# JuliaParallel/DistributedArrays.jl

Hardware: NVIDIA H100
Metric: GB/s for map! and sum on Float32 DArray (higher is better)
Workload: dtype f32

## Files before the change

distributedarrays.jl_b200/_broadcast.py:

```python
from __future__ import annotations

import ctypes as C
import struct
from typing import Callable, List, Optional, Sequence, Tuple

import numpy as np

from builtins import any as builtins_any

from . import _lib
from ._darray import B200Array, DArray, dab_dtype, darray, makelocal
from .layout import shape_of
from .runtime import close_remote_reads, open_remote_reads, runtime

_RANK = {"bool": 0, "i32": 1, "i64": 2, "i128": 3, "f32": 4, "f64": 5}


class _TagTypes(dict):

    def __missing__(self, tag):
        raise _lib.UnsupportedError(_lib.ERR_UNSUPPORTED, f"values of type {tag} have no array element type on the GPU backend "
                                    "(Int128 is served as the value type of mapreduce(f, op, d) only)")


_NPT = _TagTypes({"bool": np.dtype(np.bool_), "i32": np.dtype(np.int32), "i64": np.dtype(np.int64), "f32": np.dtype(np.float32),
                  "f64": np.dtype(np.float64), "c64": np.dtype(np.complex64), "c128": np.dtype(np.complex128)})
_TAG = {v: k for k, v in _NPT.items()}
SLICE_TRACING = [0]
_CT = {"bool": "bool", "i32": "int", "i64": "long long", "i128": "i128", "f32": "float", "f64": "double", "c64": "jl_c64", "c128": "jl_c128"}
_COMP = {"c64": "f32", "c128": "f64"}
_CPLX_OF = {"f32": "c64", "f64": "c128"}


def is_ctag(t: str) -> bool:
    return t in _COMP

# ... 498 lines not shown
    for d in range(nd):
        o = int(out_shape[d])
        ext = [sh[d] for sh in shapes]
        for e, sh in zip(ext, arg_shapes):
            if e != o and e != 1:
                raise _lib.DimensionMismatch(_lib.ERR_DIM_MISMATCH, f"arrays could not be broadcast: {tuple(sh)} vs {tuple(out_shape)}")
        if o == 1:
            continue
        if groups:
            po, pext = groups[-1]
            if all((pe == po and e == o) or (pe == 1 and e == 1) for pe, e in zip(pext, ext)):
                groups[-1] = (po * o, [pe * e for pe, e in zip(pext, ext)])
                continue
        groups.append((o, ext))
    if not groups:
        groups = [(1, [1] * len(shapes))]
    return tuple(g[0] for g in groups), [tuple(g[1][k] for g in groups) for k in range(len(shapes))]


def _dense_strides(shape):
    s, out = 1, []
    for d in shape:
        out.append(s)
        s *= int(d)
    return out


class LocalArg:

    def __init__(self, arr: Optional[B200Array] = None, scalar=None, tag: str = "f64", temp: bool = False):
        self.arr, self.scalar, self.tag, self.temp = arr, scalar, tag, temp


def run_local(rt, expr: Expr, out: B200Array, largs: List[LocalArg]):
    n = out.size
    if n == 0:
        return
    out_tag = tag_of(out.dtype)
    full = [a for a in largs if a.arr is not None]
    same = all(a.arr.shape == out.shape or a.arr.size == n and _squeeze(a.arr.shape) == _squeeze(out.shape) for a in full)
    ctx = rt.ctx
    code = dab_dtype(out.dtype)
    rt.last_kernel = "fixed"
    cplx = uses_complex(expr) or builtins_any(is_ctag(a.tag) for a in largs)
    if same and not cplx and expr.jt == out_tag and out_tag != "bool":
        x0 = largs[0] if largs and largs[0].arr is not None and largs[0].tag == out_tag else None
        if x0 is not None and all(_only_arg0(expr)):
            ab = match_affine(expr)
            if ab is not None:
                a = np.asarray(ab[0], dtype=out.dtype)
                b = np.asarray(ab[1], dtype=out.dtype)
                _lib.call("dab_affine", ctx, code, C.c_void_p(out.ptr), C.c_void_p(x0.arr.ptr), C.c_void_p(a.ctypes.data),
                          C.c_void_p(b.ctypes.data), n)
                rt.last_kernel = "dab_affine"
                return
            if expr.op in _UN and _is_arg(expr.args[0], 0):
                _lib.call("dab_unary", ctx, code, _UN[expr.op], C.c_void_p(out.ptr), C.c_void_p(x0.arr.ptr), n)
                return
            if _is_arg(expr, 0):
                _lib.call("dab_unary", ctx, code, _lib.MAP_ID, C.c_void_p(out.ptr), C.c_void_p(x0.arr.ptr), n)
                return
        if expr.op in _BIN and len(expr.args) == 2 and not (expr.op == "div" and out_tag[0] != "f"):
            l, r = expr.args
            la = largs[l.val] if l.op == "arg" else None
            ra = largs[r.val] if r.op == "arg" else None

            def arr_ok(e, a):
                return e.op == "arg" and a is not None and a.arr is not None and a.tag == out_tag

            def sc_val(e, a):
                if e.op == "const" and e.jt == out_tag:
                    return e.val
                if e.op == "arg" and a is not None and a.arr is None and a.tag == out_tag:
                    return a.scalar
                return None

            if arr_ok(l, la) and arr_ok(r, ra):
                _lib.call("dab_binary", ctx, code, _BIN[expr.op], C.c_void_p(out.ptr), C.c_void_p(la.arr.ptr), C.c_void_p(ra.arr.ptr), n)
                return
            if arr_ok(l, la) and sc_val(r, ra) is not None:
                s = np.asarray(sc_val(r, ra), dtype=out.dtype)
                _lib.call("dab_binary_scalar", ctx, code, _BIN[expr.op], C.c_void_p(out.ptr), C.c_void_p(la.arr.ptr), C.c_void_p(s.ctypes.data), 0, n)
                return
            if arr_ok(r, ra) and sc_val(l, la) is not None:
                s = np.asarray(sc_val(l, la), dtype=out.dtype)
                _lib.call("dab_binary_scalar", ctx, code, _BIN[expr.op], C.c_void_p(out.ptr), C.c_void_p(ra.arr.ptr), C.c_void_p(s.ctypes.data), 1, n)
                return
    if expr.op == "const" and expr.jt == out_tag:
        v = np.asarray(expr.val, dtype=out.dtype)
        _lib.call("dab_fill", ctx, code, C.c_void_p(out.ptr), n, C.c_void_p(v.ctypes.data))
        return
    rt.last_kernel = "dab_broadcast_expr"
    if uses_tag(expr, "i128"):
        raise _lib.UnsupportedError(_lib.ERR_UNSUPPORTED, "Int128 values are served inside mapreduce(f, op, d) only, not in a broadcast")
    if expr.jt[0] == "f" and out_tag[0] not in "fc":
        raise _lib.UnsupportedError(_lib.ERR_UNSUPPORTED, f"broadcast of {expr.jt} values into a {out_tag} destination (InexactError semantics) is not served")
    if is_ctag(expr.jt) and not is_ctag(out_tag):
        raise _lib.UnsupportedError(_lib.ERR_UNSUPPORTED, f"broadcast of {expr.jt} values into a {out_tag} destination (InexactError semantics) is not served")
    expr, largs = split_c128_scalars(expr, largs)
    src = codegen(convert(expr, out_tag)).encode()
    oshape_nd, ashapes = tuple(out.shape), {k: tuple(a.arr.shape) for k, a in enumerate(largs) if a.arr is not None}
    if len(oshape_nd) > 4 or any(len(sh) > 4 for sh in ashapes.values()):
        keys = sorted(ashapes)
        oshape_nd, coll = collapse_dims(oshape_nd, [ashapes[k] for k in keys])
        ashapes = dict(zip(keys, coll))
    oshape = _pad4(oshape_nd)
    nargs = len(largs)
    if nargs > 8:
        raise _lib.UnsupportedError(_lib.ERR_UNSUPPORTED, "more than 8 broadcast arguments are not served")
    dts = (C.c_int32 * max(nargs, 1))()
    ptrs = (C.c_void_p * max(nargs, 1))()
    strides = (C.c_size_t * (4 * max(nargs, 1)))()
    scal = (C.c_uint64 * max(nargs, 1))()
    for k, a in enumerate(largs):
        dts[k] = dab_dtype(_NPT[a.tag])
        if a.arr is not None:
            ptrs[k] = a.arr.ptr
            ash = _pad4(ashapes[k])
            dense = _dense_strides(ash)
            for d in range(4):
                if ash[d] == oshape[d]:
                    strides[4 * k + d] = dense[d]
                elif ash[d] == 1:
                    strides[4 * k + d] = 0
                else:
                    raise _lib.DimensionMismatch(_lib.ERR_DIM_MISMATCH, f"arrays could not be broadcast: {a.arr.shape} vs {out.shape}")
        else:
            ptrs[k] = None
            scal[k] = struct.unpack("<Q", np.asarray(a.scalar, dtype=_NPT[a.tag]).tobytes().ljust(8, b"\0"))[0]
    _lib.call("dab_broadcast_expr", ctx, src, code, C.c_void_p(out.ptr), _lib.sz4(oshape), _lib.sz4(_dense_strides(oshape)), nargs, dts,
              ptrs, strides, scal)


def split_c128_scalars(expr: Expr, largs: List["LocalArg"]):
    ks = [k for k, a in enumerate(largs) if a.arr is None and a.tag == "c128"]
    if not ks:
        return expr, largs
    largs, sub = list(largs), {}
    for k in ks:
        z = complex(largs[k].scalar)
        largs[k] = LocalArg(None, z.real, "f64")
        largs.append(LocalArg(None, z.imag, "f64"))
        sub[k] = Expr("complex", (Expr("arg", (), "f64", k), Expr("arg", (), "f64", len(largs) - 1)), "c128")

    def rw(e: Expr) -> Expr:
        if e.op == "arg":
            return sub.get(e.val, e)
        return Expr(e.op, tuple(rw(a) for a in e.args), e.jt, e.val, e.weak) if e.args else e

    return rw(expr), largs


def _squeeze(shape):
    return tuple(s for s in shape if s != 1)


def _only_arg0(e: Expr):
    if e.op == "arg":
        yield e.val == 0
    elif e.op != "const":
        for a in e.args:
            yield from _only_arg0(a)


# ... 24 lines not shown

def _bcview(arg_dims: Sequence[int], I) -> Tuple:
    out = []
    for k, s in enumerate(arg_dims):
        if s == 1:
            out.append((1, 1))
        elif k < len(I):
            lo, hi = I[k]
            if not (1 <= lo and hi <= s):
                raise _lib.DimensionMismatch(_lib.ERR_DIM_MISMATCH, "broadcast view could not be constructed")
            out.append((lo, hi))
        else:
            out.append((1, s))
    return tuple(out)


def _localise(rt, a, I, pid) -> LocalArg:
    if isinstance(a, DArray):
        view = _bcview(a.dims, I)
        arr = makelocal(a, view, pid)
        return LocalArg(arr, None, tag_of(a.dtype), temp=arr is not a.chunks.get(pid))
    if isinstance(a, np.ndarray) and a.ndim > 0:
        view = _bcview(a.shape, I)
        sl = a[tuple(slice(lo - 1, hi) for lo, hi in view)]
        return LocalArg(B200Array.from_numpy(rt, sl), None, tag_of(a.dtype), temp=True)
    e = Expr.wrap(a.item() if isinstance(a, np.ndarray) else a)
    return LocalArg(None, e.val, e.jt)


def _remote_args(dest_layout, args) -> List[DArray]:
    return [a for a in args if isinstance(a, DArray) and not (a.layout.pids == dest_layout.pids and a.layout.indices == dest_layout.indices)]


def _broadcast_chunks(dest: DArray, expr: Expr, args) -> DArray:
    rt = dest.rt
    fenced = open_remote_reads(rt, _remote_args(dest.layout, args), "host")
    for pid, out in dest.chunks.items():
        I = dest.layout.localindices(pid)
        largs = [_localise(rt, a, I, pid) for a in args]
        run_local(rt, expr, out, largs)
        for la in largs:
            if la.temp and la.arr is not None:
                la.arr.free()
    close_remote_reads(rt, fenced, "host")
    return dest


def _materialise_views(args):
    from ._darray import SubDArray
    out, temps = [], []
    for a in args:
        if isinstance(a, SubDArray):
            a = a.to_darray()
            temps.append(a)
        out.append(a)
    return out, temps


def broadcast_into(dest: DArray, f: Callable, *args) -> DArray:
    args, _views = _materialise_views(args)
    try:
        return _broadcast_into(dest, f, *args)
    finally:
        for v in _views:
            v.close()


def _broadcast_into(dest: DArray, f: Callable, *args) -> DArray:
    shapes = [a.dims if isinstance(a, DArray) else (a.shape if isinstance(a, np.ndarray) else ()) for a in args]
    for shp in shapes:
        for k, s in enumerate(shp):
            want = dest.dims[k] if k < len(dest.dims) else 1
            if s != 1 and s != want:
                raise _lib.DimensionMismatch(_lib.ERR_DIM_MISMATCH, f"destination axes {dest.dims} are not compatible with source axes {tuple(shp)}")
    expr = trace(f, [_arg_tag(a) for a in args])
    return _broadcast_chunks(dest, expr, args)


def broadcast(f: Callable, *args, rt=None) -> DArray:
    args, _views = _materialise_views(args)
    try:
        return _broadcast(f, *args, rt=rt)
    finally:
        for v in _views:
            v.close()


def _broadcast(f: Callable, *args, rt=None) -> DArray:
    rt = rt or next((a.rt for a in args if isinstance(a, DArray)), None) or runtime()
    shapes = [a.dims if isinstance(a, DArray) else (a.shape if isinstance(a, np.ndarray) else ()) for a in args]
    dims = _bc_shape(shapes)
    expr = trace(f, [_arg_tag(a) for a in args])
    out_dt = _NPT[expr.jt]
    dest = darray(lambda I: B200Array.empty(rt, shape_of(I), out_dt), dims, dtype=out_dt, rt=rt)
    return _broadcast_chunks(dest, expr, args)


def copy(d: DArray) -> DArray:
    from ._darray import similar
    return _broadcast_into(similar(d), lambda x: x, d)


deepcopy = copy


def drandn(dims, procs=None, dist=None, dtype=np.float64, seed: int = 1234, rt=None) -> DArray:
    from ._darray import component_dtype, drand
    dt = np.dtype(dtype)
    if dt.kind == "c":
# ... 61 lines not shown
```

distributedarrays.jl_b200/_mapreduce.py:

```python
from __future__ import annotations

import builtins
import ctypes as C
import operator
from typing import Callable, Dict, Optional, Sequence, Tuple

import numpy as np

from . import _lib
from ._broadcast import Expr, broadcast, is_ctag, tag_of, trace, _NPT
from ._darray import B200Array, DArray, component_dtype, dab_dtype, is_complex, np_dtype
from .layout import Layout, collapse_for_region, ravel, shape_of, unravel
from .runtime import close_remote_reads, exchange_stacks, fence, grouped_exchange, open_remote_reads

_OPS = {"+": _lib.SUM, "add": _lib.SUM, "sum": _lib.SUM, "*": _lib.PROD, "mul": _lib.PROD, "prod": _lib.PROD, "max": _lib.MAX,
        "min": _lib.MIN}
_OPF = {operator.add: _lib.SUM, operator.mul: _lib.PROD, builtins.max: _lib.MAX, builtins.min: _lib.MIN, np.add: _lib.SUM,
        np.multiply: _lib.PROD, np.maximum: _lib.MAX, np.minimum: _lib.MIN}


def _op_code(op) -> int:
    if isinstance(op, str) and op in _OPS:
        return _OPS[op]
    if op in _OPF:
# ... 17 lines not shown
            code = {"abs": _lib.MAP_ABS, "abs2": _lib.MAP_ABS2, "neg": _lib.MAP_NEG, "isnan": _lib.MAP_ISNAN}.get(e.op)
            if code is not None:
                return code, None, e
        return None, None, e
    if e.jt == tag and len(e.args) == 1 and e.args[0].op == "arg":
        code = {"abs": _lib.MAP_ABS, "abs2": _lib.MAP_ABS2, "neg": _lib.MAP_NEG}.get(e.op)
        if code is not None:
            return code, None, e
    if e.op == "mul" and e.jt == tag and builtins.all(a.op == "arg" for a in e.args):
        return _lib.MAP_ABS2, None, e
    if e.op in _CMPMAP:
        l, r = e.args

        def unpromote(side, const):
            if side.op == "convert" and side.args[0].op == "arg" and side.args[0].jt == tag and const.op == "const":
                c = const.val
                if tag == "f32" and const.jt == "f64" and float(np.float32(c)) == c:
                    return side.args[0], Expr("const", (), tag, c)
                if tag in ("i32", "i64") and const.jt in ("i64",) and side.jt == "i64":
                    return side.args[0], Expr("const", (), tag, c) if -2**31 <= c < 2**31 or tag == "i64" else (side, const)
            return side, const

        l, r = unpromote(l, r)
        r, l = unpromote(r, l)
        if l.op == "arg" and r.op == "const" and l.jt == tag:
            return _CMPMAP[e.op], np.asarray(r.val, dtype=np.dtype(dtype)), e
        if r.op == "arg" and l.op == "const" and r.jt == tag:
            return _CMPMAP[_FLIP[e.op]], np.asarray(l.val, dtype=np.dtype(dtype)), e
    if e.op == "isnan" and e.args[0].op == "arg":
        return _lib.MAP_ISNAN, None, e
    return None, None, e


def _result_dtype(dtype, op: int, mapc: int) -> np.dtype:
    out = C.c_int32()
    _lib.check(_lib.lib().dab_reduce_result_dtype(dab_dtype(dtype), op, mapc, C.byref(out)))
    return np.dtype(np.int64) if out.value == _lib.I64 else np_dtype(out.value)




def _gather_slots(d: DArray, launch: Callable[[int, B200Array, int], None]) -> np.ndarray:
    rt = d.rt
    wpr = rt.workers_per_rank
    slots = B200Array.empty(rt, (16 * wpr,), np.uint8, temp=True)
    try:
        for pid, ch in d.chunks.items():
            launch(pid, ch, slots.ptr + 16 * ((pid - 1) % wpr))
        if rt.world > 1:
            allslots = B200Array.empty(rt, (16 * wpr * rt.world,), np.uint8, temp=True)
            _lib.call("dab_allgather", rt.ctx, C.c_void_p(slots.ptr), C.c_void_p(allslots.ptr), 16 * wpr)
            host = allslots.to_numpy()
            allslots.free()
        else:
            host = slots.to_numpy()
    finally:
        rt.sync()
        slots.free()
    return host.view(np.uint8)


def _fold(host: np.ndarray, pids: Sequence[int], rdt: np.dtype, op: int):
    vals = np.empty(len(pids), dtype=rdt)
    for i, pid in enumerate(pids):
        vals[i] = host[16 * (pid - 1):16 * (pid - 1) + rdt.itemsize].view(rdt)[0]
    out = np.zeros(1, dtype=rdt)
    rcode = _lib.I64 if rdt == np.dtype(np.int64) else dab_dtype(rdt)
    _lib.check(_lib.lib().dab_combine_ordered(rcode, op, C.c_void_p(vals.ctypes.data), len(pids), C.c_void_p(out.ctypes.data)))
    return out[0], vals

# ... 82 lines not shown
        _lib.call("dab_mapreduce_expr", rt.ctx, src, val_code, opc_k, ch.size, n, dts, ptrs, scal, C.c_void_p(slot_ptr))

    try:
        host = _gather_slots(d, launch)
    finally:
        for t in temps:
            t.free()
        close_remote_reads(rt, fenced, "host")
    if wide:
        vals = [_int128(host[16 * (pid - 1):16 * pid].tobytes()) for pid in d.layout.pids]
        res = fold128(vals, opc)
        return (res, vals) if return_partials else res
    res, vals = _fold(host, d.layout.pids, rdt, opc if opc != _lib.COUNT else _lib.SUM)
    return (res, vals) if return_partials else res


def _mapreduce_all(f, op, d: DArray, return_partials: bool = False, others: Sequence = ()):
    opc = op if isinstance(op, int) else _op_code(op)
    if others:
        expr = trace(f, [tag_of(d.dtype)] + [_arg_tag_of(a) for a in others])
        return _mapreduce_expr(expr, opc, d, others, return_partials)
    mapc, param, expr = classify_map(f, d.dtype)
    if is_complex(d.dtype) and mapc is not None and not _complex_served(opc, mapc):
        if mapc == _lib.MAP_ID and opc in (_lib.MAX, _lib.MIN):
            raise TypeError(f"MethodError: no method matching isless(::{d.dtype}, ::{d.dtype}) -- complex numbers are not ordered")
        mapc = None
        if expr is None:
            expr = trace(lambda z: z, [tag_of(d.dtype)])
    if mapc is None:
        return _mapreduce_expr(expr, opc, d, (), return_partials)
    _check_nonempty(d, opc)
    rt = d.rt
    pp = C.c_void_p(param.ctypes.data) if param is not None else None
    rdt = _result_dtype(d.dtype, opc, mapc)
    if rt.workers_per_rank == 1 and d.layout.pids == rt.workers() and not return_partials:
        ch = d.chunks[rt.myid()]
        out = np.zeros(2, dtype=np.uint64)
        _lib.call("dab_mapreduce_all", rt.ctx, dab_dtype(d.dtype), opc, mapc, pp, C.c_void_p(ch.ptr), ch.size, C.c_void_p(out.ctypes.data))
        return out.view(np.uint8)[:rdt.itemsize].view(rdt)[0]
    code = dab_dtype(d.dtype)
    host = _gather_slots(d, lambda pid, ch, slot: _lib.call("dab_reduce", rt.ctx, code, opc, mapc, pp, C.c_void_p(ch.ptr), ch.size, C.c_void_p(slot)))
    res, vals = _fold(host, d.layout.pids, rdt, opc)
    return (res, vals) if return_partials else res


def _complex_served(opc: int, mapc: int) -> bool:
    out = C.c_int32()
    return _lib.lib().dab_reduce_result_dtype(_lib.C64, opc, mapc, C.byref(out)) == _lib.OK


def _arg_tag_of(a) -> str:
    from ._broadcast import _arg_tag
    return _arg_tag(a)


def reduce(op, d: DArray, dims=None, init=None):
    return mapreduce(None, op, d, dims=dims, init=init)


def mapreduce(f: Optional[Callable], op, d: DArray, *ds, dims=None, init=None, _partials: bool = False):
    from ._darray import SubDArray
    if isinstance(d, Expr):
        from . import _slices
        if _slices.tracing():
            return _slices.reduce_of_slice(f, op, d, ds, dims, init)
    if isinstance(d, SubDArray):
        tmp = d.to_darray()
        try:
            return mapreduce(f, op, tmp, *ds, dims=dims, init=init, _partials=_partials)
        finally:
            if dims is None:
                tmp.close()
    if dims is None:
        if init is not None:
            raise _lib.UnsupportedError(_lib.ERR_UNSUPPORTED, "mapreduce(f, op, d; init) without dims falls back to scalar iteration in the reference; not served")
        return _mapreduce_all(f, op, d, _partials, ds)
    if ds:
        tmp = broadcast(f, d, *ds)
        try:
            return mapreducedim(None, op, tmp, dims, init)
        finally:
            tmp.close()
    return mapreducedim(f, op, d, dims, init)


def sum(d: DArray, f: Optional[Callable] = None, dims=None):
    return mapreduce(f, "+", d, dims=dims)


def prod(d: DArray, f: Optional[Callable] = None, dims=None):
    return mapreduce(f, "*", d, dims=dims)


def maximum(d: DArray, f: Optional[Callable] = None, dims=None):
    return mapreduce(f, "max", d, dims=dims)


def minimum(d: DArray, f: Optional[Callable] = None, dims=None):
    return mapreduce(f, "min", d, dims=dims)


def _pred_reduce(opc: int, d: DArray, f: Optional[Callable]):
    from ._darray import SubDArray
    if isinstance(d, SubDArray):
        tmp = d.to_darray()
        try:
            return _pred_reduce(opc, tmp, f)
        finally:
            tmp.close()
    if f is None:
        if d.dtype != np.dtype(np.bool_):
            raise TypeError("TypeError: non-boolean used in boolean context")
        return _mapreduce_all(None, opc, d)
    mapc, param, e = classify_map(f, d.dtype)
    if e is not None and e.jt != "bool":
        raise TypeError("TypeError: non-boolean used in boolean context")
    return _mapreduce_all(f, opc, d)


def _count_dims(d: DArray, f: Optional[Callable], dims) -> Tuple[DArray, int]:
    from ._broadcast import ifelse
    from ._darray import SubDArray
    if isinstance(d, SubDArray):
        tmp = d.to_darray()
        try:
            return _count_dims(tmp, f, dims)
        finally:
            tmp.close()
    if f is None and d.dtype != np.dtype(np.bool_):
        raise TypeError("TypeError: non-boolean used in boolean context")
    pred = (lambda x: x) if f is None else f
# ... 331 lines not shown
```

distributedarrays.jl_b200/csrc/dab_comm.cu:

```cuda
#include <dlfcn.h>
#include <nccl.h>

#include "dab_common.cuh"
#include "dab_scalar_ops.cuh"

namespace {

struct NcclApi {
    void* handle = nullptr;
    ncclResult_t (*GetUniqueId)(ncclUniqueId*) = nullptr;
    ncclResult_t (*CommInitRank)(ncclComm_t*, int, ncclUniqueId, int) = nullptr;
    ncclResult_t (*CommDestroy)(ncclComm_t) = nullptr;
    ncclResult_t (*AllGather)(const void*, void*, size_t, ncclDataType_t, ncclComm_t, cudaStream_t) = nullptr;
    ncclResult_t (*AllReduce)(const void*, void*, size_t, ncclDataType_t, ncclRedOp_t, ncclComm_t, cudaStream_t) = nullptr;
    ncclResult_t (*Send)(const void*, size_t, ncclDataType_t, int, ncclComm_t, cudaStream_t) = nullptr;
    ncclResult_t (*Recv)(void*, size_t, ncclDataType_t, int, ncclComm_t, cudaStream_t) = nullptr;
    ncclResult_t (*GroupStart)() = nullptr;
    ncclResult_t (*GroupEnd)() = nullptr;
    const char* (*GetErrorString)(ncclResult_t) = nullptr;
    const char* (*GetLastError)(ncclComm_t) = nullptr;
    bool ok = false;
    char why[256] = "";
};

NcclApi& nccl() {
    static NcclApi api;
    static bool tried = false;
    if (tried) return api;
    tried = true;
    const char* names[] = {"libnccl.so.2", "libnccl.so", nullptr};
    for (int i = 0; names[i] && !api.handle; ++i) api.handle = dlopen(names[i], RTLD_NOW | RTLD_GLOBAL);
    if (!api.handle) {
        snprintf(api.why, sizeof(api.why), "dlopen(libnccl.so.2) failed: %s", dlerror());
        return api;
// ... 149 lines not shown
        default: return dab_fail(ctx, DAB_ERR_ARG, "dab_allreduce: bad op %d", op);
    }
    DAB_NCCL(ctx, api.AllReduce(send_dev, recv_dev, count, dt, ro, (ncclComm_t)ctx->comm, ctx->stream));
    ctx->launches++;
    return DAB_OK;
}

int32_t dab_group_start(dab_ctx* ctx) {
    DAB_ENTER(ctx);
    NEED_COMM(ctx);
    DAB_NCCL(ctx, api.GroupStart());
    return DAB_OK;
}
int32_t dab_group_end(dab_ctx* ctx) {
    DAB_ENTER(ctx);
    NEED_COMM(ctx);
    DAB_NCCL(ctx, api.GroupEnd());
    ctx->launches++;
    return DAB_OK;
}
int32_t dab_send(dab_ctx* ctx, const void* send_dev, size_t nbytes, int32_t peer) {
    DAB_ENTER(ctx);
    NEED_COMM(ctx);
    DAB_NCCL(ctx, api.Send(send_dev, nbytes, ncclInt8, peer, (ncclComm_t)ctx->comm, ctx->stream));
    return DAB_OK;
}
int32_t dab_recv(dab_ctx* ctx, void* recv_dev, size_t nbytes, int32_t peer) {
    DAB_ENTER(ctx);
    NEED_COMM(ctx);
    DAB_NCCL(ctx, api.Recv(recv_dev, nbytes, ncclInt8, peer, (ncclComm_t)ctx->comm, ctx->stream));
    return DAB_OK;
}

int32_t dab_mapreduce_all(dab_ctx* ctx, int32_t dtype, int32_t op, int32_t map, const void* map_param, const void* x, size_t n,
                          void* out_host) {
    DAB_ENTER_NOFLUSH(ctx);
    int32_t rdt;
    if (!out_host || op == DAB_EXTREMA || dab_reduce_result_dtype(dtype, op, map, &rdt) != DAB_OK) {
        DAB_FLUSH(ctx);
        DAB_REQUIRE(ctx, out_host, DAB_ERR_ARG, "dab_mapreduce_all: null out");
        if (op == DAB_EXTREMA) return dab_fail(ctx, DAB_ERR_UNSUPPORTED, "dab_mapreduce_all: extrema combines through dab_reduce + dab_allgather");
        return dab_fail(ctx, DAB_ERR_ARG, "bad dtype/op");
    }
    const bool cplx = rdt == DAB_C64 || rdt == DAB_C128;
    if ((ctx->mbox_ranks > 1 || !ctx->comm || ctx->nranks == 1) && n > 0 && !cplx) {
        ctx->fuse_op = op;
        int32_t st = dab_reduce(ctx, dtype, op, map, map_param, x, n, ctx->result_slot);
        ctx->fuse_op = -1;
        if (st != DAB_OK) return st;
        DAB_CUDA(ctx, cudaStreamSynchronize(ctx->stream));
        const volatile unsigned long long* h = (const volatile unsigned long long*)ctx->host_slot;
        if (h[1] != 0) return dab_fail(ctx, DAB_ERR_NCCL, "fused combine timed out waiting for a peer's chunk result (did every rank call?)");
        unsigned long long bits = h[0];
        memset(out_host, 0, 8);
        memcpy(out_host, &bits, dab_dtype_size(rdt));
        return DAB_OK;
    }
    if (cplx && ctx->mbox_ranks > 1 && !ctx->comm) {
        DAB_FLUSH(ctx);
        return dab_fail(ctx, DAB_ERR_UNSUPPORTED, "dab_mapreduce_all: a complex result across %d ranks needs the NCCL communicator "
                        "(the mailbox combine carries 8-byte results)", ctx->mbox_ranks);
    }
    int32_t st = dab_reduce(ctx, dtype, op, map, map_param, x, n, ctx->result_slot);
    if (st != DAB_OK) return st;
    const int P = ctx->comm ? ctx->nranks : 1;
    const void* src = ctx->result_slot;
    if (P > 1) {
        NEED_COMM(ctx);
        DAB_NCCL(ctx, api.AllGather(ctx->result_slot, ctx->gather_slots, 16, ncclInt8, (ncclComm_t)ctx->comm, ctx->stream));
        ctx->launches++;
        src = ctx->gather_slots;
    }
    DAB_CUDA(ctx, cudaMemcpyAsync(ctx->host_slot, src, (size_t)P * 16, cudaMemcpyDeviceToHost, ctx->stream));
    DAB_CUDA(ctx, cudaStreamSynchronize(ctx->stream));
    unsigned char tmp[DAB_MAX_RANKS * 16];
    size_t es = dab_dtype_size(rdt);
    for (int i = 0; i < P; ++i) memcpy(tmp + (size_t)i * es, (const char*)ctx->host_slot + (size_t)i * 16, es);
    unsigned char res[16] = {0};
    st = dab_combine_ordered(rdt, op, tmp, (size_t)P, res);
    if (st != DAB_OK) return dab_fail(ctx, st, "%s", dab_last_error(nullptr));
    memset(out_host, 0, es > 8 ? es : 8);
    memcpy(out_host, res, es);
    return DAB_OK;
}
// ... 126 lines not shown
```

distributedarrays.jl_b200/csrc/dab_common.cuh:

```cuda
#pragma once
#include <cuda_runtime.h>

#include <cstdint>
#include <cstdio>
#include <cstring>

#include "../../include/dab200.h"

#define DAB_MAX_REDUCE_BLOCKS 262144
#define DAB_SLOT_BYTES 64
#define DAB_MAX_RANKS 64

struct dab_pending_affine {
    int active;
    int32_t dtype;
    void* y;
    const void* x;
    size_t n;
    unsigned char a[8], b[8];
};

struct dab_ctx {
    int device;
    int sm_count;
    cudaStream_t stream;
    void* block_partials;
    unsigned int* counter;
    void* result_slot;
    void* gather_slots;
    void* host_slot;
    void* dim_scratch;
    size_t dim_scratch_bytes;
    uint64_t launches;
    void* comm;
    int rank, nranks;
    void* mailbox;
    void** peer_mbox_dev;
    void* peer_mbox_host[DAB_MAX_RANKS];
    int mbox_ranks;
    unsigned long long mbox_seq;
    unsigned long long barrier_seq;
    int fuse_op;
    struct dab_alloc_cache* cache;
    void* sort_dev;
    size_t sort_dev_bytes;
    void* stage[2];
    cudaEvent_t stage_ev[2];
    void* sort_host;
    unsigned long long sort_epoch;
    long long opt_combine_timeout_ms;
    long long opt_gemm_kc;
    int opt_gemm_rawhi;
    int opt_gemm_simt;
    int opt_gemv_phase;
    int opt_gemv_t_cols;
    int opt_gemv_t_waves;
    int opt_ew_tma;
    dab_pending_affine pending;
    int defer_off;
    char err[512];
};

extern thread_local char dab_tls_err[512];

int32_t dab_fail(dab_ctx* ctx, int32_t status, const char* fmt, ...);
int32_t dab_fail_cuda(dab_ctx* ctx, cudaError_t e, const char* what, const char* file, int line);

#define DAB_CUDA(ctx, call)                                                             \
    do {                                                                                \
        cudaError_t e__ = (call);                                                       \
        if (e__ != cudaSuccess) return dab_fail_cuda((ctx), e__, #call, __FILE__, __LINE__); \
    } while (0)

#define DAB_REQUIRE(ctx, cond, status, ...)                          \
// ... 16 lines not shown
        if ((ctx) == nullptr) return dab_fail(nullptr, DAB_ERR_ARG, "null ctx"); \
        DAB_CUDA((ctx), cudaSetDevice((ctx)->device));                      \
        DAB_FLUSH(ctx);                                                     \
    } while (0)

#define DAB_ENTER_NOFLUSH(ctx)                                              \
    do {                                                                    \
        if ((ctx) == nullptr) return dab_fail(nullptr, DAB_ERR_ARG, "null ctx"); \
        DAB_CUDA((ctx), cudaSetDevice((ctx)->device));                      \
    } while (0)

#define DAB_LAUNCHED(ctx)                          \
    do {                                           \
        (ctx)->launches++;                         \
        DAB_CUDA((ctx), cudaGetLastError());       \
    } while (0)

static inline size_t dab_dtype_size(int32_t dt) {
    switch (dt) {
        case DAB_F32: return 4;
        case DAB_F64: return 8;
        case DAB_I32: return 4;
        case DAB_I64: return 8;
        case DAB_U8: return 1;
        case DAB_C64: return 8;
        case DAB_C128: return 16;
        default: return 0;
    }
}

#define DAB_MBOX_SLOT 32
#define DAB_MBOX_BARRIER_OFFSET (2 * DAB_MAX_RANKS * DAB_MBOX_SLOT)
#define DAB_MBOX_BYTES (DAB_MBOX_BARRIER_OFFSET + DAB_MAX_RANKS * 8)
struct FusedComm {
    void* const* peers;
    void* host_out;
    unsigned long long seq;
    unsigned long long timeout_ns;
    int rank, nranks, op;
};

__device__ __forceinline__ unsigned long long dab_globaltimer_ns() {
    unsigned long long t;
    asm volatile("mov.u64 %0, %globaltimer;" : "=l"(t));
    return t;
}
__device__ __forceinline__ int4 ld_stream(const int4* p) { return __ldcs(p); }
__device__ __forceinline__ void st_stream(int4* p, int4 v) { __stcs(p, v); }

template <typename T>
struct alignas(16) Pack {
    static constexpr int N = 16 / sizeof(T);
    T v[N];
};

template <typename T>
struct alignas(2 * sizeof(T)) Cplx {
    T re, im;
};

template <typename T>
__device__ __forceinline__ Pack<T> as_pack(int4 r) {
    Pack<T> p;
    memcpy(&p, &r, 16);
    return p;
}
template <typename T>
__device__ __forceinline__ int4 as_int4(const Pack<T>& p) {
    int4 r;
// ... 25 lines not shown
```

distributedarrays.jl_b200/csrc/dab_core.cu:

```cuda
#include <cstdarg>
#include <cstdlib>
#include <map>
#include <mutex>
#include <new>
#include <thread>
#include <unordered_map>

#include "dab_common.cuh"

thread_local char dab_tls_err[512] = "";

struct dab_alloc_cache {
    std::unordered_map<void*, size_t> live;
    std::multimap<size_t, void*> free_blocks;
    size_t cached_bytes = 0;
    static constexpr size_t kMaxBlock = 16ull << 30;
    static constexpr size_t kMaxCached = 32ull << 30;
};

int dab_resident_ctas(const void* kernel, int threads) {
    static std::mutex mu;
    static std::unordered_map<const void*, int> cache;
    std::lock_guard<std::mutex> lk(mu);
    auto it = cache.find(kernel);
// ... 75 lines not shown
    ctx->opt_gemv_t_waves = 4;
    ctx->opt_gemv_t_cols = 8;
    ctx->cache = new (std::nothrow) dab_alloc_cache();
#define INIT_CUDA(call)                                                     \
    do {                                                                    \
        cudaError_t e__ = (call);                                           \
        if (e__ != cudaSuccess) {                                           \
            int32_t st = dab_fail_cuda(nullptr, e__, #call, __FILE__, __LINE__); \
            delete ctx;                                                     \
            return st;                                                      \
        }                                                                   \
    } while (0)
    INIT_CUDA(cudaSetDevice(device));
    cudaDeviceProp prop;
    INIT_CUDA(cudaGetDeviceProperties(&prop, device));
    if (prop.major != 9 || prop.minor != 0) {
        delete ctx;
        return dab_fail(nullptr, DAB_ERR_UNSUPPORTED, "device %d is sm_%d%d; libdab200 is built for sm_90a only", device,
                        prop.major, prop.minor);
    }
    ctx->sm_count = prop.multiProcessorCount;
    INIT_CUDA(cudaStreamCreateWithFlags(&ctx->stream, cudaStreamNonBlocking));
    {
        cudaMemPool_t pool;
        INIT_CUDA(cudaDeviceGetDefaultMemPool(&pool, device));
        unsigned long long keep = ~0ull;
        INIT_CUDA(cudaMemPoolSetAttribute(pool, cudaMemPoolAttrReleaseThreshold, &keep));
    }
    INIT_CUDA(cudaMalloc(&ctx->block_partials, ((size_t)DAB_MAX_REDUCE_BLOCKS + DAB_MAX_REDUCE_BLOCKS / 256 + 16) * 16));
    INIT_CUDA(cudaMalloc((void**)&ctx->counter, (DAB_MAX_REDUCE_BLOCKS / 256 + 16) * 4));
    INIT_CUDA(cudaMemsetAsync(ctx->counter, 0, (DAB_MAX_REDUCE_BLOCKS / 256 + 16) * 4, ctx->stream));
    INIT_CUDA(cudaMalloc(&ctx->result_slot, DAB_SLOT_BYTES));
    INIT_CUDA(cudaMalloc(&ctx->gather_slots, (size_t)DAB_MAX_RANKS * 16));
    INIT_CUDA(cudaHostAlloc(&ctx->host_slot, (size_t)(DAB_MAX_RANKS + 2) * 16, cudaHostAllocDefault));
    INIT_CUDA(cudaStreamSynchronize(ctx->stream));
    memset(ctx->host_slot, 0, (size_t)(DAB_MAX_RANKS + 2) * 16);
#undef INIT_CUDA
    *out = ctx;
    return DAB_OK;
}

int32_t dab_comm_destroy(dab_ctx* ctx);
int32_t dab_mailbox_detach(dab_ctx* ctx);

int32_t dab_shutdown(dab_ctx* ctx) {
    if (!ctx) return DAB_OK;
    cudaSetDevice(ctx->device);
    const int32_t st = dab_flush_pending(ctx);
    cudaStreamSynchronize(ctx->stream);
    if (ctx->comm) dab_comm_destroy(ctx);
    cudaFree(ctx->block_partials);
    cudaFree(ctx->counter);
    cudaFree(ctx->result_slot);
    cudaFree(ctx->gather_slots);
    if (ctx->dim_scratch) cudaFree(ctx->dim_scratch);
    if (ctx->sort_dev) cudaFree(ctx->sort_dev);
    if (ctx->sort_host) cudaFreeHost(ctx->sort_host);
    for (int b = 0; b < 2; ++b)
        if (ctx->stage[b]) {
            cudaFreeHost(ctx->stage[b]);
            cudaEventDestroy(ctx->stage_ev[b]);
        }
    if (ctx->cache) {
        for (auto& kv : ctx->cache->free_blocks) cudaFree(kv.second);
        delete ctx->cache;
        ctx->cache = nullptr;
    }
    dab_mailbox_detach(ctx);
    cudaFreeHost(ctx->host_slot);
// ... 363 lines not shown
```

distributedarrays.jl_b200/csrc/dab_reduce.cu:

```cuda
#include <type_traits>

#include <cmath>

#include "dab_reduce_traits.cuh"

namespace {

constexpr int RD_UNROLL = 4;

struct NoStore {
    template <typename T>
    __device__ __forceinline__ void vec(Pack<T>&, size_t) const {}
    template <typename T>
    __device__ __forceinline__ T scalar(T v, size_t) const { return v; }
};
template <typename T>
struct AffineStore {
    AffineF<T> f;
    T* y;
    int4* yv;
    __device__ __forceinline__ void vec(Pack<T>& p, size_t i) const {
#pragma unroll
        for (int k = 0; k < Pack<T>::N; ++k) p.v[k] = f(p.v[k]);
        st_stream(yv + i, as_int4(p));
// ... 94 lines not shown
    v = block_reduce<R>(v, smem);
    if (threadIdx.x == 0) {
        counter[1 + g] = 0;
        gpartials[g] = v;
        __threadfence();
        unsigned int ticket = atomicAdd(counter, 1u);
        is_last = (ticket == ngroups - 1);
    }
    __syncthreads();
    if (!is_last) return;
    __threadfence();
    A fin = R::identity();
    for (unsigned int i = threadIdx.x; i < ngroups; i += RD_THREADS) fin = R::comb(fin, gpartials[i]);
    fin = block_reduce<R>(fin, smem);
    if (threadIdx.x == 0) {
        *counter = 0;
        if constexpr (std::is_arithmetic<A>::value) {
            Out res;
            if (finalize_mode == 1) res = (Out)(fin == (A)n_for_all);
            else if (finalize_mode == 2) res = (Out)(fin != (A)0);
            else res = (Out)fin;
            memcpy(out, &res, sizeof(Out));
            if (sizeof(Out) < 8) memset((char*)out + sizeof(Out), 0, 8 - sizeof(Out));
            A wide = fin;
            memcpy((char*)out + 8, &wide, sizeof(A));
            if (sizeof(A) < 8) memset((char*)out + 8 + sizeof(A), 0, 8 - sizeof(A));
            if (fc.host_out && fc.nranks <= 1) {
                unsigned long long bits = 0;
                memcpy(&bits, &res, sizeof(Out));
                volatile unsigned long long* h = reinterpret_cast<volatile unsigned long long*>(fc.host_out);
                h[0] = bits;
                h[1] = 0ull;
                __threadfence_system();
            }
        } else if constexpr (is_cplx<Out>::value) {
            using CT = decltype(Out::re);
            const Out res{(CT)fin.re, (CT)fin.im};
            memset(out, 0, 16);
            memcpy(out, &res, sizeof(Out));
        } else {
            memset(out, 0, 16);
            memcpy(out, &fin, sizeof(A));
        }
    }
    if constexpr (!std::is_arithmetic<Out>::value) return;
    else {
    if (fc.nranks <= 1) return;
    __shared__ unsigned long long pay[2];
    __shared__ unsigned long long got[DAB_MAX_RANKS];
    __shared__ int timed_out;
    if (threadIdx.x == 0) {
        memcpy(&pay[0], out, 8);
        memcpy(&pay[1], (char*)out + 8, 8);
        timed_out = 0;
    }
    __syncthreads();
    const size_t bank = (size_t)(fc.seq & 1ull) * DAB_MAX_RANKS * DAB_MBOX_SLOT;
    if (threadIdx.x < (unsigned)fc.nranks) {
        volatile unsigned long long* dst =
            reinterpret_cast<volatile unsigned long long*>((char*)fc.peers[threadIdx.x] + bank + (size_t)fc.rank * DAB_MBOX_SLOT);
        dst[0] = pay[0];
        dst[1] = pay[1];
        __threadfence_system();
        dst[2] = fc.seq;
        volatile unsigned long long* src =
            reinterpret_cast<volatile unsigned long long*>((char*)fc.peers[fc.rank] + bank + (size_t)threadIdx.x * DAB_MBOX_SLOT);
        const unsigned long long t0 = dab_globaltimer_ns();
        unsigned int spins = 0;
        while (src[2] != fc.seq) {
            if ((++spins & 1023u) == 0 && dab_globaltimer_ns() - t0 > fc.timeout_ns) {
                timed_out = 1;
                break;
            }
        }
        __threadfence_system();
        got[threadIdx.x] = src[0];
    }
    __syncthreads();
    if (threadIdx.x == 0) {
        Out a;
        memcpy(&a, &got[0], sizeof(Out));
        for (int j = 1; j < fc.nranks; ++j) {
            Out b;
            memcpy(&b, &got[j], sizeof(Out));
            switch (fc.op) {
                case DAB_SUM: case DAB_COUNT: a = jl::add(a, b); break;
                case DAB_PROD: a = jl::mul(a, b); break;
                case DAB_MAX: a = jl::max(a, b); break;
                case DAB_MIN: a = jl::min(a, b); break;
                case DAB_ALL: a = (Out)(a != (Out)0 && b != (Out)0); break;
                default: a = (Out)(a != (Out)0 || b != (Out)0); break;
            }
        }
        unsigned long long bits = 0;
        memcpy(&bits, &a, sizeof(Out));
        volatile unsigned long long* h = reinterpret_cast<volatile unsigned long long*>(fc.host_out);
        h[0] = bits;
        h[1] = (unsigned long long)timed_out;
        __threadfence_system();
    }
    }
}

template <typename T, typename Map, typename R, typename Out, typename St = NoStore>
int32_t launch_reduce(dab_ctx* ctx, const T* x, size_t n, Map map, void* out, int finalize_mode, St st = St()) {
    constexpr int VPT = 16 / sizeof(T);
    size_t head = ((16 - ((uintptr_t)x & 15)) & 15) / sizeof(T);
    if (head > n) head = n;
    if constexpr (!std::is_same<St, NoStore>::value) st.yv = reinterpret_cast<int4*>(st.y + head);
    size_t tiles = (n - head) / ((size_t)VPT * RD_THREADS * RD_UNROLL);
    size_t k = 2;
    if ((tiles + k - 1) / k > (size_t)DAB_MAX_REDUCE_BLOCKS) k = (tiles + DAB_MAX_REDUCE_BLOCKS - 1) / DAB_MAX_REDUCE_BLOCKS;
    size_t grid = (tiles + k - 1) / k;
    if (grid < 1) grid = 1;
    FusedComm fc;
    memset(&fc, 0, sizeof(fc));
    if (ctx->fuse_op >= 0 && ctx->mbox_ranks > 1) {
        fc.peers = ctx->peer_mbox_dev;
        fc.host_out = ctx->host_slot;
        fc.seq = ++ctx->mbox_seq;
        fc.timeout_ns = (unsigned long long)ctx->opt_combine_timeout_ms * 1000000ull;
        fc.rank = ctx->rank;
        fc.nranks = ctx->mbox_ranks;
        fc.op = ctx->fuse_op;
    } else if (ctx->fuse_op >= 0) {
        fc.host_out = ctx->host_slot;
        fc.nranks = 1;
        fc.op = ctx->fuse_op;
    }
    reduce_kernel<T, Map, R, Out, St><<<(unsigned)grid, RD_THREADS, 0, ctx->stream>>>(x, n, head, map, (typename R::A*)ctx->block_partials,
                                                                                      ctx->counter, out, finalize_mode, (long long)n, (int)k, fc, st);
    DAB_LAUNCHED(ctx);
    return DAB_OK;
}

template <typename T>
using ResultOfSum = typename std::conditional<std::is_floating_point<T>::value, T, long long>::type;

template <typename T, int FN>
int32_t reduce_arith(dab_ctx* ctx, int32_t op, const T* x, size_t n, void* out) {
    MapF<T, FN> map{(T)0};
    switch (op) {
        case DAB_SUM: return launch_reduce<T, MapF<T, FN>, SumTraits<T>, ResultOfSum<T>>(ctx, x, n, map, out, 0);
        case DAB_PROD: return launch_reduce<T, MapF<T, FN>, ProdTraits<T>, ResultOfSum<T>>(ctx, x, n, map, out, 0);
        case DAB_MAX: return launch_reduce<T, MapF<T, FN>, MaxTraits<T>, T>(ctx, x, n, map, out, 0);
        case DAB_MIN: return launch_reduce<T, MapF<T, FN>, MinTraits<T>, T>(ctx, x, n, map, out, 0);
        case DAB_EXTREMA:
            if constexpr (FN == DAB_MAP_ID) return launch_reduce<T, ExtMapF<T>, ExtremaTraits<T>, Pair<T>>(ctx, x, n, ExtMapF<T>{(T)0}, out, 0);
            else return dab_fail(ctx, DAB_ERR_UNSUPPORTED, "extrema with a map is not served (no host fallback)");
        default: return dab_fail(ctx, DAB_ERR_UNSUPPORTED, "reduce op %d needs a predicate map (no host fallback)", op);
    }
}

template <typename T, int FN>
int32_t reduce_pred(dab_ctx* ctx, int32_t op, const T* x, size_t n, const void* param, void* out) {
    PredF<T, FN> map{param ? *(const T*)param : (T)0};
    int mode;
    switch (op) {
        case DAB_ALL: mode = 1; break;
        case DAB_ANY: mode = 2; break;
        case DAB_COUNT:
// ... 355 lines not shown
```

Baseline: 4286.

## Memoize broadcast launch plans and traces, fast-path whole-array reductions with spin-wait

Records the sequence of native kernel launches made by a broadcast and replays it on later calls. Replay is keyed by the function's code, its captured scalar values, the layout identity and the chunk pointers, so Python tracing and dispatch are skipped. It also caches traced expressions and reduction result dtypes. It adds a direct path for whole-array sum/prod/max/min. The fused reduction now signals completion through a sequence word in pinned host memory, which the host polls instead of calling cudaStreamSynchronize. The risks are stale plans if an id or pointer is reused, and added CPU busy-waiting.

```diff
diff --git a/distributedarrays.jl_b200/_broadcast.py b/distributedarrays.jl_b200/_broadcast.py
--- a/distributedarrays.jl_b200/_broadcast.py
+++ b/distributedarrays.jl_b200/_broadcast.py
@@ -2,6 +2,7 @@
 
 import ctypes as C
 import struct
+from types import FunctionType
 from typing import Callable, List, Optional, Sequence, Tuple
 
 import numpy as np
@@ -566,14 +567,19 @@
         self.arr, self.scalar, self.tag, self.temp = arr, scalar, tag, temp
 
 
-def run_local(rt, expr: Expr, out: B200Array, largs: List[LocalArg]):
+def _launch(rt, record: Optional[list], name: str, cargs: tuple, keep: tuple = ()):
+    _lib.call(name, rt.ctx, *cargs)
+    if record is not None:
+        record.append((name, cargs, keep, rt.last_kernel))
+
+
+def run_local(rt, expr: Expr, out: B200Array, largs: List[LocalArg], record: Optional[list] = None):
     n = out.size
     if n == 0:
         return
     out_tag = tag_of(out.dtype)
     full = [a for a in largs if a.arr is not None]
     same = all(a.arr.shape == out.shape or a.arr.size == n and _squeeze(a.arr.shape) == _squeeze(out.shape) for a in full)
-    ctx = rt.ctx
     code = dab_dtype(out.dtype)
     rt.last_kernel = "fixed"
     cplx = uses_complex(expr) or builtins_any(is_ctag(a.tag) for a in largs)
@@ -584,15 +590,15 @@
             if ab is not None:
                 a = np.asarray(ab[0], dtype=out.dtype)
                 b = np.asarray(ab[1], dtype=out.dtype)
-                _lib.call("dab_affine", ctx, code, C.c_void_p(out.ptr), C.c_void_p(x0.arr.ptr), C.c_void_p(a.ctypes.data),
-                          C.c_void_p(b.ctypes.data), n)
                 rt.last_kernel = "dab_affine"
+                _launch(rt, record, "dab_affine", (code, C.c_void_p(out.ptr), C.c_void_p(x0.arr.ptr), C.c_void_p(a.ctypes.data),
+                                                   C.c_void_p(b.ctypes.data), n), (a, b))
                 return
             if expr.op in _UN and _is_arg(expr.args[0], 0):
-                _lib.call("dab_unary", ctx, code, _UN[expr.op], C.c_void_p(out.ptr), C.c_void_p(x0.arr.ptr), n)
+                _launch(rt, record, "dab_unary", (code, _UN[expr.op], C.c_void_p(out.ptr), C.c_void_p(x0.arr.ptr), n))
                 return
             if _is_arg(expr, 0):
-                _lib.call("dab_unary", ctx, code, _lib.MAP_ID, C.c_void_p(out.ptr), C.c_void_p(x0.arr.ptr), n)
+                _launch(rt, record, "dab_unary", (code, _lib.MAP_ID, C.c_void_p(out.ptr), C.c_void_p(x0.arr.ptr), n))
                 return
         if expr.op in _BIN and len(expr.args) == 2 and not (expr.op == "div" and out_tag[0] != "f"):
             l, r = expr.args
@@ -610,19 +616,21 @@
                 return None
 
             if arr_ok(l, la) and arr_ok(r, ra):
-                _lib.call("dab_binary", ctx, code, _BIN[expr.op], C.c_void_p(out.ptr), C.c_void_p(la.arr.ptr), C.c_void_p(ra.arr.ptr), n)
+                _launch(rt, record, "dab_binary", (code, _BIN[expr.op], C.c_void_p(out.ptr), C.c_void_p(la.arr.ptr), C.c_void_p(ra.arr.ptr), n))
                 return
             if arr_ok(l, la) and sc_val(r, ra) is not None:
                 s = np.asarray(sc_val(r, ra), dtype=out.dtype)
-                _lib.call("dab_binary_scalar", ctx, code, _BIN[expr.op], C.c_void_p(out.ptr), C.c_void_p(la.arr.ptr), C.c_void_p(s.ctypes.data), 0, n)
+                _launch(rt, record, "dab_binary_scalar", (code, _BIN[expr.op], C.c_void_p(out.ptr), C.c_void_p(la.arr.ptr), C.c_void_p(s.ctypes.data),
+                                                          0, n), (s,))
                 return
             if arr_ok(r, ra) and sc_val(l, la) is not None:
                 s = np.asarray(sc_val(l, la), dtype=out.dtype)
-                _lib.call("dab_binary_scalar", ctx, code, _BIN[expr.op], C.c_void_p(out.ptr), C.c_void_p(ra.arr.ptr), C.c_void_p(s.ctypes.data), 1, n)
+                _launch(rt, record, "dab_binary_scalar", (code, _BIN[expr.op], C.c_void_p(out.ptr), C.c_void_p(ra.arr.ptr), C.c_void_p(s.ctypes.data),
+                                                          1, n), (s,))
                 return
     if expr.op == "const" and expr.jt == out_tag:
         v = np.asarray(expr.val, dtype=out.dtype)
-        _lib.call("dab_fill", ctx, code, C.c_void_p(out.ptr), n, C.c_void_p(v.ctypes.data))
+        _launch(rt, record, "dab_fill", (code, C.c_void_p(out.ptr), n, C.c_void_p(v.ctypes.data)), (v,))
         return
     rt.last_kernel = "dab_broadcast_expr"
     if uses_tag(expr, "i128"):
@@ -662,8 +670,8 @@
         else:
             ptrs[k] = None
             scal[k] = struct.unpack("<Q", np.asarray(a.scalar, dtype=_NPT[a.tag]).tobytes().ljust(8, b"\0"))[0]
-    _lib.call("dab_broadcast_expr", ctx, src, code, C.c_void_p(out.ptr), _lib.sz4(oshape), _lib.sz4(_dense_strides(oshape)), nargs, dts,
-              ptrs, strides, scal)
+    _launch(rt, record, "dab_broadcast_expr", (src, code, C.c_void_p(out.ptr), _lib.sz4(oshape), _lib.sz4(_dense_strides(oshape)), nargs, dts,
+                                               ptrs, strides, scal))
 
 
 def split_c128_scalars(expr: Expr, largs: List["LocalArg"]):
@@ -754,17 +762,21 @@
     return [a for a in args if isinstance(a, DArray) and not (a.layout.pids == dest_layout.pids and a.layout.indices == dest_layout.indices)]
 
 
-def _broadcast_chunks(dest: DArray, expr: Expr, args) -> DArray:
+def _broadcast_chunks(dest: DArray, expr: Expr, args, record: Optional[list] = None) -> DArray:
     rt = dest.rt
     fenced = open_remote_reads(rt, _remote_args(dest.layout, args), "host")
     for pid, out in dest.chunks.items():
         I = dest.layout.localindices(pid)
         largs = [_localise(rt, a, I, pid) for a in args]
-        run_local(rt, expr, out, largs)
+        run_local(rt, expr, out, largs, record)
         for la in largs:
             if la.temp and la.arr is not None:
                 la.arr.free()
+                if record is not None:
+                    record.append(None)
     close_remote_reads(rt, fenced, "host")
+    if fenced and record is not None:
+        record.append(None)
     return dest
 
 
@@ -779,24 +791,109 @@
     return out, temps
 
 
+_MEMO_MAX = 256
+_TRACES: dict = {}
+_PLANS: dict = {}
+
+
+def _value_key(v):
+    t = type(v)
+    if t is bool or t is int:
+        return t, v
+    if t is float:
+        return t, struct.pack("<d", v)
+    if t is complex:
+        return t, struct.pack("<dd", v.real, v.imag)
+    if isinstance(v, (np.number, np.bool_)):
+        return t, v.tobytes()
+    return None
+
+
+def _closure_key(f):
+    if type(f) is not FunctionType or f.__code__.co_names or f.__kwdefaults__:
+        return None
+    vals = []
+    for c in f.__closure__ or ():
+        try:
+            k = _value_key(c.cell_contents)
+        except ValueError:
+            return None
+        if k is None:
+            return None
+        vals.append(k)
+    for v in f.__defaults__ or ():
+        k = _value_key(v)
+        if k is None:
+            return None
+        vals.append(k)
+    return f.__code__, tuple(vals)
+
+
+def _memo_put(memo: dict, key, value):
+    if len(memo) >= _MEMO_MAX:
+        memo.clear()
+    memo[key] = value
+
+
+def _trace_memo(f: Callable, tags: List[str]) -> Expr:
+    ck = _closure_key(f)
+    if ck is None:
+        return trace(f, tags)
+    key = (ck, tuple(tags))
+    e = _TRACES.get(key)
+    if e is None:
+        e = trace(f, tags)
+        _memo_put(_TRACES, key, e)
+    return e
+
+
+def _plan_key(dest: DArray, f: Callable, args):
+    ck = _closure_key(f)
+    if ck is None:
+        return None
+    fps = []
+    for a in (dest,) + args:
+        if type(a) is DArray:
+            fps.append((id(a.layout), a.dtype, tuple(ch.ptr for ch in a.chunks.values())))
+        else:
+            k = _value_key(a)
+            if k is None:
+                return None
+            fps.append(k)
+    return ck, tuple(fps)
+
+
 def broadcast_into(dest: DArray, f: Callable, *args) -> DArray:
+    key = _plan_key(dest, f, args) if type(dest) is DArray else None
+    plan = _PLANS.get(key) if key is not None else None
+    if plan is not None:
+        rt = dest.rt
+        for name, cargs, _keep, kernel in plan[0]:
+            rt.last_kernel = kernel
+            _lib.call(name, rt.ctx, *cargs)
+        return dest
     args, _views = _materialise_views(args)
+    record = [] if key is not None else None
     try:
-        return _broadcast_into(dest, f, *args)
+        _broadcast_into(dest, f, *args, record=record)
     finally:
         for v in _views:
             v.close()
-
-
-def _broadcast_into(dest: DArray, f: Callable, *args) -> DArray:
+    if record is not None and None not in record:
+        layouts = tuple(a.layout for a in (dest, *args) if type(a) is DArray)
+        _memo_put(_PLANS, key, (record, layouts))
+    return dest
+
+
+def _broadcast_into(dest: DArray, f: Callable, *args, record: Optional[list] = None) -> DArray:
     shapes = [a.dims if isinstance(a, DArray) else (a.shape if isinstance(a, np.ndarray) else ()) for a in args]
     for shp in shapes:
         for k, s in enumerate(shp):
             want = dest.dims[k] if k < len(dest.dims) else 1
             if s != 1 and s != want:
                 raise _lib.DimensionMismatch(_lib.ERR_DIM_MISMATCH, f"destination axes {dest.dims} are not compatible with source axes {tuple(shp)}")
-    expr = trace(f, [_arg_tag(a) for a in args])
-    return _broadcast_chunks(dest, expr, args)
+    expr = _trace_memo(f, [_arg_tag(a) for a in args])
+    return _broadcast_chunks(dest, expr, args, record)
 
 
 def broadcast(f: Callable, *args, rt=None) -> DArray:
diff --git a/distributedarrays.jl_b200/_mapreduce.py b/distributedarrays.jl_b200/_mapreduce.py
--- a/distributedarrays.jl_b200/_mapreduce.py
+++ b/distributedarrays.jl_b200/_mapreduce.py
@@ -73,10 +73,17 @@
     return None, None, e
 
 
+_RDT: Dict[Tuple[np.dtype, int, int], np.dtype] = {}
+
+
 def _result_dtype(dtype, op: int, mapc: int) -> np.dtype:
-    out = C.c_int32()
-    _lib.check(_lib.lib().dab_reduce_result_dtype(dab_dtype(dtype), op, mapc, C.byref(out)))
-    return np.dtype(np.int64) if out.value == _lib.I64 else np_dtype(out.value)
+    key = (np.dtype(dtype), op, mapc)
+    rdt = _RDT.get(key)
+    if rdt is None:
+        out = C.c_int32()
+        _lib.check(_lib.lib().dab_reduce_result_dtype(dab_dtype(dtype), op, mapc, C.byref(out)))
+        rdt = _RDT[key] = np.dtype(np.int64) if out.value == _lib.I64 else np_dtype(out.value)
+    return rdt
 
 
 
@@ -225,16 +232,35 @@
     _check_nonempty(d, opc)
     rt = d.rt
     pp = C.c_void_p(param.ctypes.data) if param is not None else None
+    if rt.workers_per_rank == 1 and d.layout.pids == rt.workers() and not return_partials:
+        return _reduce_all_one_call(d, opc, mapc, pp)
     rdt = _result_dtype(d.dtype, opc, mapc)
-    if rt.workers_per_rank == 1 and d.layout.pids == rt.workers() and not return_partials:
-        ch = d.chunks[rt.myid()]
-        out = np.zeros(2, dtype=np.uint64)
-        _lib.call("dab_mapreduce_all", rt.ctx, dab_dtype(d.dtype), opc, mapc, pp, C.c_void_p(ch.ptr), ch.size, C.c_void_p(out.ctypes.data))
-        return out.view(np.uint8)[:rdt.itemsize].view(rdt)[0]
     code = dab_dtype(d.dtype)
     host = _gather_slots(d, lambda pid, ch, slot: _lib.call("dab_reduce", rt.ctx, code, opc, mapc, pp, C.c_void_p(ch.ptr), ch.size, C.c_void_p(slot)))
     res, vals = _fold(host, d.layout.pids, rdt, opc)
     return (res, vals) if return_partials else res
+
+
+def _reduce_all_one_call(d: DArray, opc: int, mapc: int, pp=None):
+    rt = d.rt
+    ch = d.chunks[rt.myid()]
+    rdt = _result_dtype(d.dtype, opc, mapc)
+    out = np.zeros(2, dtype=np.uint64)
+    _lib.call("dab_mapreduce_all", rt.ctx, dab_dtype(d.dtype), opc, mapc, pp, C.c_void_p(ch.ptr), ch.size, C.c_void_p(out.ctypes.data))
+    return out.view(rdt)[0]
+
+
+def _whole_array_fast(d, opc: int):
+    if type(d) is not DArray:
+        return None
+    rt = d.rt
+    if rt.workers_per_rank != 1 or d.layout.pids != rt.workers():
+        return None
+    if opc in (_lib.MAX, _lib.MIN):
+        if is_complex(d.dtype):
+            return None
+        _check_nonempty(d, opc)
+    return _reduce_all_one_call(d, opc, _lib.MAP_ID)
 
 
 def _complex_served(opc: int, mapc: int) -> bool:
@@ -278,18 +304,34 @@
 
 
 def sum(d: DArray, f: Optional[Callable] = None, dims=None):
+    if f is None and dims is None:
+        r = _whole_array_fast(d, _lib.SUM)
+        if r is not None:
+            return r
     return mapreduce(f, "+", d, dims=dims)
 
 
 def prod(d: DArray, f: Optional[Callable] = None, dims=None):
+    if f is None and dims is None:
+        r = _whole_array_fast(d, _lib.PROD)
+        if r is not None:
+            return r
     return mapreduce(f, "*", d, dims=dims)
 
 
 def maximum(d: DArray, f: Optional[Callable] = None, dims=None):
+    if f is None and dims is None:
+        r = _whole_array_fast(d, _lib.MAX)
+        if r is not None:
+            return r
     return mapreduce(f, "max", d, dims=dims)
 
 
 def minimum(d: DArray, f: Optional[Callable] = None, dims=None):
+    if f is None and dims is None:
+        r = _whole_array_fast(d, _lib.MIN)
+        if r is not None:
+            return r
     return mapreduce(f, "min", d, dims=dims)
 
 
diff --git a/distributedarrays.jl_b200/csrc/dab_comm.cu b/distributedarrays.jl_b200/csrc/dab_comm.cu
--- a/distributedarrays.jl_b200/csrc/dab_comm.cu
+++ b/distributedarrays.jl_b200/csrc/dab_comm.cu
@@ -1,5 +1,7 @@
 #include <dlfcn.h>
 #include <nccl.h>
+
+#include <atomic>
 
 #include "dab_common.cuh"
 #include "dab_scalar_ops.cuh"
@@ -215,6 +217,34 @@
     return DAB_OK;
 }
 
+namespace {
+
+inline void cpu_relax() {
+#if defined(__x86_64__) || defined(__i386__)
+    __builtin_ia32_pause();
+#elif defined(__aarch64__)
+    asm volatile("yield" ::: "memory");
+#endif
+}
+
+int32_t wait_done(dab_ctx* ctx, const volatile unsigned long long* word, unsigned long long seq) {
+    for (unsigned int spins = 1;; ++spins) {
+        if (*word == seq) break;
+        cpu_relax();
+        if ((spins & 4095u) != 0) continue;
+        const cudaError_t q = cudaStreamQuery(ctx->stream);
+        if (q == cudaErrorNotReady) continue;
+        if (q == cudaSuccess && *word == seq) break;
+        DAB_CUDA(ctx, cudaStreamSynchronize(ctx->stream));
+        if (*word == seq) break;
+        return dab_fail(ctx, DAB_ERR_CUDA, "fused reduction %llu finished without writing its completion word", seq);
+    }
+    std::atomic_thread_fence(std::memory_order_acquire);
+    return DAB_OK;
+}
+
+}
+
 int32_t dab_mapreduce_all(dab_ctx* ctx, int32_t dtype, int32_t op, int32_t map, const void* map_param, const void* x, size_t n,
                           void* out_host) {
     DAB_ENTER_NOFLUSH(ctx);
@@ -231,8 +261,9 @@
         int32_t st = dab_reduce(ctx, dtype, op, map, map_param, x, n, ctx->result_slot);
         ctx->fuse_op = -1;
         if (st != DAB_OK) return st;
-        DAB_CUDA(ctx, cudaStreamSynchronize(ctx->stream));
-        const volatile unsigned long long* h = (const volatile unsigned long long*)ctx->host_slot;
+        const volatile unsigned long long* h = (const volatile unsigned long long*)((char*)ctx->host_slot + DAB_HOST_DONE_OFFSET);
+        st = wait_done(ctx, h + 2, ctx->done_seq);
+        if (st != DAB_OK) return st;
         if (h[1] != 0) return dab_fail(ctx, DAB_ERR_NCCL, "fused combine timed out waiting for a peer's chunk result (did every rank call?)");
         unsigned long long bits = h[0];
         memset(out_host, 0, 8);
diff --git a/distributedarrays.jl_b200/csrc/dab_common.cuh b/distributedarrays.jl_b200/csrc/dab_common.cuh
--- a/distributedarrays.jl_b200/csrc/dab_common.cuh
+++ b/distributedarrays.jl_b200/csrc/dab_common.cuh
@@ -40,6 +40,7 @@
     int mbox_ranks;
     unsigned long long mbox_seq;
     unsigned long long barrier_seq;
+    unsigned long long done_seq;
     int fuse_op;
     struct dab_alloc_cache* cache;
     void* sort_dev;
@@ -122,9 +123,12 @@
 #define DAB_MBOX_SLOT 32
 #define DAB_MBOX_BARRIER_OFFSET (2 * DAB_MAX_RANKS * DAB_MBOX_SLOT)
 #define DAB_MBOX_BYTES (DAB_MBOX_BARRIER_OFFSET + DAB_MAX_RANKS * 8)
+#define DAB_HOST_DONE_OFFSET ((DAB_MAX_RANKS + 2) * 16)
+#define DAB_HOST_SLOT_BYTES ((DAB_MAX_RANKS + 4) * 16)
 struct FusedComm {
     void* const* peers;
     void* host_out;
+    unsigned long long done_seq;
     unsigned long long seq;
     unsigned long long timeout_ns;
     int rank, nranks, op;
diff --git a/distributedarrays.jl_b200/csrc/dab_core.cu b/distributedarrays.jl_b200/csrc/dab_core.cu
--- a/distributedarrays.jl_b200/csrc/dab_core.cu
+++ b/distributedarrays.jl_b200/csrc/dab_core.cu
@@ -131,9 +131,9 @@
     INIT_CUDA(cudaMemsetAsync(ctx->counter, 0, (DAB_MAX_REDUCE_BLOCKS / 256 + 16) * 4, ctx->stream));
     INIT_CUDA(cudaMalloc(&ctx->result_slot, DAB_SLOT_BYTES));
     INIT_CUDA(cudaMalloc(&ctx->gather_slots, (size_t)DAB_MAX_RANKS * 16));
-    INIT_CUDA(cudaHostAlloc(&ctx->host_slot, (size_t)(DAB_MAX_RANKS + 2) * 16, cudaHostAllocDefault));
+    INIT_CUDA(cudaHostAlloc(&ctx->host_slot, DAB_HOST_SLOT_BYTES, cudaHostAllocDefault));
     INIT_CUDA(cudaStreamSynchronize(ctx->stream));
-    memset(ctx->host_slot, 0, (size_t)(DAB_MAX_RANKS + 2) * 16);
+    memset(ctx->host_slot, 0, DAB_HOST_SLOT_BYTES);
 #undef INIT_CUDA
     *out = ctx;
     return DAB_OK;
diff --git a/distributedarrays.jl_b200/csrc/dab_reduce.cu b/distributedarrays.jl_b200/csrc/dab_reduce.cu
--- a/distributedarrays.jl_b200/csrc/dab_reduce.cu
+++ b/distributedarrays.jl_b200/csrc/dab_reduce.cu
@@ -150,6 +150,7 @@
                 h[0] = bits;
                 h[1] = 0ull;
                 __threadfence_system();
+                h[2] = fc.done_seq;
             }
         } else if constexpr (is_cplx<Out>::value) {
             using CT = decltype(Out::re);
@@ -216,6 +217,7 @@
         h[0] = bits;
         h[1] = (unsigned long long)timed_out;
         __threadfence_system();
+        h[2] = fc.done_seq;
     }
     }
 }
@@ -233,18 +235,18 @@
     if (grid < 1) grid = 1;
     FusedComm fc;
     memset(&fc, 0, sizeof(fc));
+    if (ctx->fuse_op >= 0) {
+        fc.host_out = (char*)ctx->host_slot + DAB_HOST_DONE_OFFSET;
+        fc.done_seq = ++ctx->done_seq;
+        fc.op = ctx->fuse_op;
+        fc.nranks = 1;
+    }
     if (ctx->fuse_op >= 0 && ctx->mbox_ranks > 1) {
         fc.peers = ctx->peer_mbox_dev;
-        fc.host_out = ctx->host_slot;
         fc.seq = ++ctx->mbox_seq;
         fc.timeout_ns = (unsigned long long)ctx->opt_combine_timeout_ms * 1000000ull;
         fc.rank = ctx->rank;
         fc.nranks = ctx->mbox_ranks;
-        fc.op = ctx->fuse_op;
-    } else if (ctx->fuse_op >= 0) {
-        fc.host_out = ctx->host_slot;
-        fc.nranks = 1;
-        fc.op = ctx->fuse_op;
     }
     reduce_kernel<T, Map, R, Out, St><<<(unsigned)grid, RD_THREADS, 0, ctx->stream>>>(x, n, head, map, (typename R::A*)ctx->block_partials,
                                                                                       ctx->counter, out, finalize_mode, (long long)n, (int)k, fc, st);
```

Measured after the change: 4323, median of 6. About the same (+0.9%).
